# ShingoNishimoto/gnss_sim_receiver

Measured on AMD Instinct MI355X. Metric: IF Msamples/sec processed & tracked-channels sustained @1/2/4/8 GPU, higher is better.
Workload: dtype f32

## Files before the change

### gnss_sim_receiver_amd/csrc/trk_fast.hip

```cpp
#include <algorithm>
#include <cstdlib>
#include <type_traits>

#include "code_bits.h"
#include "corr_device.h"
#include "trk_engine.h"

#ifdef GNSSHIP_CORR_PROFILE
namespace gnsship {
namespace {
constexpr int kFProfEpochs = 16;
constexpr int kFProfFirst = 8;
constexpr int kFProfSlots = 88;
__device__ unsigned long long* g_trkf_prof = nullptr;
__shared__ int g_fprof_epoch;
__shared__ unsigned long long g_fprof_lds[kFProfEpochs * kFProfSlots];
#ifndef GNSSHIP_PROF_MASK
#define GNSSHIP_PROF_MASK 0xffffffffffffffffull
#endif
__device__ __forceinline__ constexpr bool prof_on(int k) { return ((GNSSHIP_PROF_MASK) >> (k < 63 ? k : 63)) & 1ull; }
__device__ __forceinline__ void trkf_prof_stamp(int e, int k)
{
    if (!prof_on(k)) return;
    const int r = e - kFProfFirst;
// ... 75 lines not shown
constexpr int acc_waves() { return (2 * NTT + 3) / 4; }
template <int NTT, int W>
constexpr int n_producers() { return W - 2 - acc_waves<NTT>(); }
constexpr int kMaxAccWaves = 4;
static_assert(kFWaves - 4 >= 1 && GNSSHIP_THRU_WAVES - 4 >= 1, "trk_fast needs at least one producer wave");
constexpr int kRoleControl = 0, kRoleReplay = 1, kRoleProducer = 2, kRoleAccum = 3;
#define GNSSHIP_PROBE(NAME)                                                  \
    do {                                                                     \
        _Pragma("unroll") for (int pr_ = 0; pr_ < (NAME); pr_++) __builtin_amdgcn_s_sleep(4); \
    } while (0)
#ifndef GNSSHIP_DELAY_ACC
#define GNSSHIP_DELAY_ACC 0
#endif
#ifndef GNSSHIP_DELAY_PROD
#define GNSSHIP_DELAY_PROD 0
#endif
#ifndef GNSSHIP_DELAY_REPLAY
#define GNSSHIP_DELAY_REPLAY 0
#endif
#ifndef GNSSHIP_DELAY_LOOP
#define GNSSHIP_DELAY_LOOP 0
#endif
#ifndef GNSSHIP_POLL_SLEEP
#define GNSSHIP_POLL_SLEEP 0
#endif
constexpr uint64_t kSlotEmpty = ~0ull;

struct FJob {
    int64_t off;
    float rem_code, code_step;
    float shifts[5];
    float dz_re, dz_im;
    float rem_carr, step;
    int32_t runnable, in_margin, M, S, tail, pad;
};

struct SpecArgs {
    double step_d, rate;
    int64_t if_num;
    float rem_prev;
    int32_t n_pred;
};

struct SpecPred {
    float rem, step, dz_re, dz_im;
};

struct FShared {
    FJob job;
    float taps[2][2 * kMaxTaps + 2];
    int32_t taps_seq[kMaxAccWaves];
    gnsship_trk_dump_record drec;
    double coh;
    int32_t seed_seq;
    int32_t job_seq;
    int32_t pre_seq;
    int32_t lock_seq;
    int32_t locked;
    int32_t tail_seq;
    int32_t acc_groups[kMaxAccWaves];
    int32_t step_seq;
    SpecArgs spec;
    SpecPred pred;
    int32_t pred_seq;
    int32_t verdict;
    f2 tailp[kAvxLanes][kMaxTaps + 1];
    double pre_pll[2], pre_dll[2];
    int32_t pll_seq, dll_seq;
};

__device__ __forceinline__ float unif(float v) { return __builtin_bit_cast(float, __builtin_amdgcn_readfirstlane(__builtin_bit_cast(int, v))); }
__device__ __forceinline__ FJob uniform_job(const FJob& s)
{
    FJob j;
    const uint64_t off = static_cast<uint64_t>(s.off);
    j.off = static_cast<int64_t>((static_cast<uint64_t>(static_cast<uint32_t>(__builtin_amdgcn_readfirstlane(static_cast<int>(off >> 32)))) << 32) |
                                 static_cast<uint32_t>(__builtin_amdgcn_readfirstlane(static_cast<int>(off & 0xffffffffu))));
    j.rem_code = unif(s.rem_code);
    j.code_step = unif(s.code_step);
    for (int t = 0; t < 5; t++) j.shifts[t] = unif(s.shifts[t]);
    j.dz_re = unif(s.dz_re);
    j.dz_im = unif(s.dz_im);
    j.rem_carr = unif(s.rem_carr);
    j.step = unif(s.step);
    j.runnable = __builtin_amdgcn_readfirstlane(s.runnable);
    j.in_margin = __builtin_amdgcn_readfirstlane(s.in_margin);
    j.M = __builtin_amdgcn_readfirstlane(s.M);
    j.S = __builtin_amdgcn_readfirstlane(s.S);
    j.tail = __builtin_amdgcn_readfirstlane(s.tail);
    j.pad = 0;
    return j;
}

__device__ __forceinline__ void store_slot(uint64_t* p, f2 z) { __hip_atomic_store(p, __builtin_bit_cast(uint64_t, z), __ATOMIC_RELAXED, __HIP_MEMORY_SCOPE_WORKGROUP); }
__device__ __forceinline__ uint64_t load_slot(const uint64_t* p) { return __hip_atomic_load(p, __ATOMIC_RELAXED, __HIP_MEMORY_SCOPE_WORKGROUP); }

__device__ __forceinline__ void publish_seq(int32_t* p, int v)
{
    __builtin_amdgcn_fence(__ATOMIC_RELEASE, "workgroup");
    __hip_atomic_store(p, v, __ATOMIC_RELAXED, __HIP_MEMORY_SCOPE_WORKGROUP);
}
__device__ __forceinline__ void wait_seq(int32_t* p, int need)
{
    while (__hip_atomic_load(p, __ATOMIC_RELAXED, __HIP_MEMORY_SCOPE_WORKGROUP) < need) __builtin_amdgcn_s_sleep(GNSSHIP_POLL_SLEEP);
    __builtin_amdgcn_fence(__ATOMIC_ACQUIRE, "workgroup");
}

__device__ __forceinline__ void lds_release_store(int32_t* p, int v)
{
    asm volatile("s_waitcnt lgkmcnt(0)" ::: "memory");
    __hip_atomic_store(p, v, __ATOMIC_RELAXED, __HIP_MEMORY_SCOPE_WORKGROUP);
}
__device__ __forceinline__ void lds_wait_eq(const int32_t* p, int v)
{
    while (__hip_atomic_load(p, __ATOMIC_RELAXED, __HIP_MEMORY_SCOPE_WORKGROUP) != v) __builtin_amdgcn_s_sleep(GNSSHIP_POLL_SLEEP);
    asm volatile("" ::: "memory");
}
__device__ __forceinline__ void lds_wait_ge(const int32_t* p, int v)
{
    while (__hip_atomic_load(p, __ATOMIC_RELAXED, __HIP_MEMORY_SCOPE_WORKGROUP) < v) __builtin_amdgcn_s_sleep(GNSSHIP_POLL_SLEEP);
    asm volatile("" ::: "memory");
}

// ... 688 lines not shown
    const int tail = N - kAvxLanes * M;
    const int n_groups = (S + 3) / 4;
    RChan rc;
    if (role == kRoleControl) rchan_load(sc, &sc, rc);
    KFast kf = make_kfast(k, sc.geo);
    __shared__ uint32_t sec_bits[kTrkMaxSecondary / 32], dsec_bits[kTrkMaxSecondary / 32];
    if constexpr (!THRU) {
        if (tid < kTrkMaxSecondary / 32) {
            sec_bits[tid] = kf.sv.secondary_bits[tid];
            dsec_bits[tid] = kf.sv.data_secondary_bits[tid];
        }
        kf.sv.secondary_bits = sec_bits;
        kf.sv.data_secondary_bits = dsec_bits;
        __syncthreads();
    }
    const auto& kp = loop_params<THRU>(k, kf);
    const bool pre_disc = __builtin_amdgcn_readfirstlane(GNSSHIP_PRE_DISC && !k.sync[sc.geo].secondary && k.sync[sc.geo].extend == 1 ? 1 : 0) != 0;
    uint64_t seed_start = 0;
    const uint64_t vl = k.conf.vector_length;
    const float spcf = static_cast<float>(k.code_samples_per_chip);
    const int32_t has_if = k.has_if;
    const double if_step = k.if_step_rad;
    float shv_w[5], shv_n[5];
    float smin_w = 0.0f, smax_w = 0.0f, smin_n = 0.0f, smax_n = 0.0f;
#pragma unroll
    for (int t = 0; t < 5; t++) {
        shv_w[t] = t < NT ? k.shifts[t] : 0.0f;
        shv_n[t] = t < NT ? k.shifts_n[t] : 0.0f;
        smin_w = fminf(smin_w, shv_w[t]);
        smax_w = fmaxf(smax_w, shv_w[t]);
        smin_n = fminf(smin_n, shv_n[t]);
        smax_n = fmaxf(smax_n, shv_n[t]);
    }
    auto code_fields = [&](FJob& j, uint64_t nir) __attribute__((always_inline)) {
        const bool nw = uni(rc.narrow) != 0;
        j.off = static_cast<int64_t>(nir - buf_first);
        j.rem_code = __fmul_rn(static_cast<float>(rc.rem_code_phase_chips), spcf);
        j.code_step = __fmul_rn(static_cast<float>(rc.code_phase_step_chips), spcf);
#pragma unroll
        for (int t = 0; t < 5; t++) j.shifts[t] = nw ? shv_n[t] : shv_w[t];
        const float smin = nw ? smin_n : smin_w, smax = nw ? smax_n : smax_w;
        const double span = static_cast<double>(j.code_step) * static_cast<double>(N > 0 ? N - 1 : 0);
        const double lo = fmin(0.0, span) + smin - j.rem_code - 2.0;
        const double hi = fmax(0.0, span) + smax - j.rem_code + 2.0;
        j.in_margin = (isfinite(lo) && isfinite(hi) && lo >= -kCodeMargin && hi < static_cast<double>(L + kCodeMargin)) ? 1 : 0;
        j.M = M;
        j.S = S;
        j.tail = tail;
    };
    auto make_seed = [&](int e) {
        const bool runnable = e < max_rounds && (rc.state == 2 || rc.state == 3 || rc.state == 4) && rc.nitems_read >= buf_first &&
                              rc.nitems_read + vl <= buf_first + static_cast<uint64_t>(buf_len);
        const float rem_carr = has_if ? static_cast<float>(fmod_2pi(static_cast<double>(rc.rem_carr_phase_rad) + kTwoPi * rc.if_cyc))
                                      : rc.rem_carr_phase_rad;
        const float stepf = static_cast<float>(rc.carrier_phase_step_rad + if_step);
        if (runnable) rc.epoch_start = rc.nitems_read;
        seed_start = rc.epoch_start;
        if (lane == 0) {
            FJob& j = sh.job;
            j.runnable = runnable ? 1 : 0;
            if (runnable) {
                code_fields(j, rc.nitems_read);
                j.rem_carr = rem_carr;
                j.step = stepf;
            }
            int code = 3;
            if (!SRING && __hip_atomic_load(&sh.pred_seq, __ATOMIC_RELAXED, __HIP_MEMORY_SCOPE_WORKGROUP) >= e + 1) {
                __builtin_amdgcn_fence(__ATOMIC_ACQUIRE, "workgroup");
                code = 2;
                if (runnable && __builtin_bit_cast(uint32_t, sh.pred.rem) == __builtin_bit_cast(uint32_t, rem_carr) &&
                    __builtin_bit_cast(uint32_t, sh.pred.step) == __builtin_bit_cast(uint32_t, stepf)) {
                    j.dz_re = sh.pred.dz_re;
                    j.dz_im = sh.pred.dz_im;
                    code = 1;
                }
            }
            sh.verdict = 4 * (e + 1) + code;
            publish_seq(&sh.seed_seq, e + 1);
            if (code == 1) publish_seq(&sh.job_seq, e + 1);
        }
    };
    if (role == kRoleControl) make_seed(0);
    int e_done = 0;
    bool cancel = false;
    if (role == kRoleReplay) {
        for (int e = 0;; e++) {
            FJob job;
                bool spec = false;
                SpecArgs sp{};
                while (__hip_atomic_load(&sh.seed_seq, __ATOMIC_RELAXED, __HIP_MEMORY_SCOPE_WORKGROUP) < e + 1) {
                    if (__hip_atomic_load(&sh.step_seq, __ATOMIC_RELAXED, __HIP_MEMORY_SCOPE_WORKGROUP) >= e + 1) {
                        sp.step_d = __builtin_bit_cast(double, uni64(__builtin_bit_cast(uint64_t, sh.spec.step_d)));
                        sp.rate = __builtin_bit_cast(double, uni64(__builtin_bit_cast(uint64_t, sh.spec.rate)));
                        sp.if_num = static_cast<int64_t>(uni64(static_cast<uint64_t>(sh.spec.if_num)));
                        sp.rem_prev = __builtin_bit_cast(float, __builtin_amdgcn_readfirstlane(__builtin_bit_cast(int, sh.spec.rem_prev)));
                        sp.n_pred = __builtin_amdgcn_readfirstlane(sh.spec.n_pred);
                        spec = true;
                        break;
                    }
                    __builtin_amdgcn_s_sleep(GNSSHIP_POLL_SLEEP);
                }
                __builtin_amdgcn_fence(__ATOMIC_ACQUIRE, "workgroup");
                GNSSHIP_FSTAMP(e, 0);
    #ifdef GNSSHIP_CORR_PROFILE
                if (lane == 0) g_fprof_epoch = e;
    #endif
                f2 zinit = f2{0.0f, 0.0f}, inc = f2{1.0f, 0.0f}, dz = f2{1.0f, 0.0f};
                float step_pre = 0.0f;
                bool published = false;
                float xl = 0.0f;
                if (spec) step_pre = static_cast<float>(sp.step_d + if_step);
                if (SRING && spec) derive_step(step_pre, inc, dz);
                if (!SRING && spec) {
                    float rem_pred = carr_rem_next(sp.rem_prev, carr_advance(sp.step_d, sp.rate, static_cast<double>(sp.n_pred)));
                    if (has_if) {
                        const int64_t ifn = (sp.if_num + kp.if_mod * static_cast<int64_t>(sp.n_pred)) % kp.fs_int;
                        const double ifc = static_cast<double>(ifn) / static_cast<double>(kp.fs_int);
                        rem_pred = static_cast<float>(fmod_2pi(static_cast<double>(rem_pred) + kTwoPi * ifc));
                    }
                    derive_all(step_pre, rem_pred, lane, inc, dz, zinit);
                    GNSSHIP_FSTAMP(e, 35);
                    GNSSHIP_PROBE(GNSSHIP_DELAY_REPLAY);
                    if (lane == 0) {
                        sh.pred.rem = rem_pred;
                        sh.pred.step = step_pre;
                        sh.pred.dz_re = dz.x;
                        sh.pred.dz_im = dz.y;
                        publish_seq(&sh.pred_seq, e + 1);
                    }
                    xl = (lane & 1) ? zinit.y : zinit.x;
                    if (lane < 2 * kAvxLanes) xl = fast_replay<G, false>(xl, dz.x, (lane & 1) ? dz.y : -dz.y, M, S, tail, Zs, rs, lane);
                    GNSSHIP_FSTAMP(e, 34);
                    wait_seq(&sh.seed_seq, e + 1);
                    const int v = __builtin_amdgcn_readfirstlane(sh.verdict);
                    int status = (v >> 2) == e + 1 ? (v & 3) : 3;
                    if (status == 3) {
                        const FJob sd = uniform_job(sh.job);
                        status = 2;
                        if (sd.runnable && __builtin_bit_cast(uint32_t, sd.step) == __builtin_bit_cast(uint32_t, step_pre) &&
                            __builtin_bit_cast(uint32_t, sd.rem_carr) == __builtin_bit_cast(uint32_t, rem_pred)) {
                            if (lane == 0) {
                                sh.job.dz_re = dz.x;
                                sh.job.dz_im = dz.y;
                                publish_seq(&sh.job_seq, e + 1);
                            }
                            status = 1;
                        }
                    }
                    GNSSHIP_FVAL(e, 78, static_cast<unsigned long long>(status));
                    if (status == 1) {
                        published = true;
                    } else {
                        for (int i = lane; i < S * kAvxLanes; i += kWave) Zs[i] = kSlotEmpty;
                    }
                    GNSSHIP_FSTAMP(e, 36);
                }
                if (!published) {
                    wait_seq(&sh.seed_seq, e + 1);
                    const FJob sd = uniform_job(sh.job);
                    if (sd.runnable) {
                        if (!(spec && __builtin_bit_cast(uint32_t, sd.step) == __builtin_bit_cast(uint32_t, step_pre))) derive_step(sd.step, inc, dz);
                        zinit = derive_chains(sd.rem_carr, inc, lane);
                        if (lane == 0) {
                            sh.job.dz_re = dz.x;
                            sh.job.dz_im = dz.y;
                        }
                    }
                    if (lane == 0) publish_seq(&sh.job_seq, e + 1);
                    if (!sd.runnable) break;
                }
                GNSSHIP_FSTAMP(e, 1);
                GNSSHIP_FCLK(e, 12);
                job = uniform_job(sh.job);
                if (!published) {
                    xl = (lane & 1) ? zinit.y : zinit.x;
                    if (lane < 2 * kAvxLanes) xl = fast_replay<G, SRING>(xl, job.dz_re, (lane & 1) ? job.dz_im : -job.dz_im, M, S, tail, Zs, rs, lane);
                }
                if (tail > 0) {
                    const i4v span = sample_span<FMT>(samples, job.off, N);
                    const f2 zl = f2{__builtin_bit_cast(float, __builtin_amdgcn_readlane(__builtin_bit_cast(int, xl), 0)),
                        __builtin_bit_cast(float, __builtin_amdgcn_readlane(__builtin_bit_cast(int, xl), 1))};
                    if (lane == 0) {
                        f2 p = normalise_avx(zl);
                        for (int j = 0; j < tail; j++) {
                            tailz[j] = p;
                            p = cmul_exact(p, inc);
                        }
                    }
                    if (job.in_margin)
                        fast_tail_products<FMT, NT, DATA, true, PACKED>(job, span, c0, c1, L, tailz, lane, sh.tailp);
                    else
                        fast_tail_products<FMT, NT, DATA, false, PACKED>(job, span, c0, c1, L, tailz, lane, sh.tailp);
                    if (lane == 0) publish_seq(&sh.tail_seq, e + 1);
                }
                GNSSHIP_FSTAMP(e, 2);
                GNSSHIP_FCLK(e, 13);
        }
    } else if (role == kRoleProducer) {
        f2 xa[G < 8 ? G : 8];
        float cv[G][NTT];
        for (int e = 0;; e++) {
            const int gbase = e * n_groups;
            wait_seq(&sh.job_seq, e + 1);
            const FJob job = uniform_job(sh.job);
            if (!job.runnable) break;
            const i4v span = sample_span<FMT>(samples, job.off, N);
            if (job.in_margin)
                fast_produce<FMT, NT, DATA, true, G, kFWaves, PACKED>(job, span, c0, c1, L, Zs, rs, Pp, rg, ready, sh.acc_groups, gbase, lane, pw, e, xa, cv);
            else
                fast_produce<FMT, NT, DATA, false, G, kFWaves, PACKED>(job, span, c0, c1, L, Zs, rs, Pp, rg, ready, sh.acc_groups, gbase, lane, pw, e, xa, cv);
            if (pw < 2) GNSSHIP_FSTAMP(e, 3 + pw);
            if (pw == 0) {
                wait_seq(&sh.pre_seq, e + 1);
                const double coh = sh.coh;
                if (lane == 0) {
                    GNSSHIP_TRK_LOOP_STAMP(8);
                    sh.locked = (coh > 0.0 && !lock_status(k, sc, coh)) ? 0 : 1;
                    GNSSHIP_TRK_LOOP_STAMP(26);
                    publish_seq(&sh.lock_seq, e + 1);
                }
            }
        }
    } else if (role == kRoleAccum) {
        for (int e = 0;; e++) {
            const int gbase = e * n_groups;
            wait_seq(&sh.job_seq, e + 1);
            const FJob job = uniform_job(sh.job);
            if (!job.runnable) break;
            {
                constexpr int NS = acc_slots<NTT>();
                float acc[NS];
                GNSSHIP_FSTAMP(e, 27);
                fast_accumulate<NTT, G>(Pp, rg, ready, &sh.acc_groups[pw], gbase, S, lane, pw, acc, e);
                GNSSHIP_FSTAMP(e, 5);
                const int r = lane >> 4;
    #pragma unroll
                for (int kk = 0; kk < NS; kk++) acc[kk] = avx_chain_sum(acc[kk]);
                if (job.tail > 0) {
                    wait_seq(&sh.tail_seq, e + 1);
                    for (int j = 0; j < job.tail; j++) {
    #pragma unroll
                        for (int kk = 0; kk < NS; kk++) {
                            const int sl = min(acc_slot<NTT>(pw, r, kk), 2 * NTT - 1);
                            const f2 tv = sh.tailp[j][sl >> 1];
                            acc[kk] = acc[kk] + ((sl & 1) ? tv.y : tv.x);
                        }
                    }
                }
                if ((lane & 15) == 0) {
    #pragma unroll
                    for (int kk = 0; kk < NS; kk++) {
                        const int sl = acc_slot<NTT>(pw, r, kk);
                        if (sl < 2 * NTT) {
                            const int tap = sl >> 1;
                            const int o = (DATA && tap == NT) ? 2 * kMaxTaps : 2 * tap;
                            sh.taps[e & 1][o + (sl & 1)] = acc[kk];
                        }
                    }
                }
                if (lane == 0) lds_release_store(&sh.taps_seq[pw], e + 1);
                if (pre_disc && pw < 2) {
#pragma unroll
                    for (int a = 0; a < NA; a++) wait_seq(&sh.taps_seq[a], e + 1);
                    const float* tp = sh.taps[e & 1];
                    const int eo = k.veml ? 2 : 0;
                    auto own = [&](int i) { return __fadd_rn(0.0f, __fmul_rn(1.0f, tp[i])); };
                    if (pw == 0 || NA == 1) {
                        const double v = pll_error_hz(k.track_pilot ? 0 : 1, own(eo + 2), own(eo + 3));
                        if (lane == 0) {
                            sh.pre_pll[e & 1] = v;
                            publish_seq(&sh.pll_seq, e + 1);
                        }
                    }
                    if (pw == 1 || NA == 1) {
                        const float ve[2] = {k.veml ? own(0) : 0.0f, k.veml ? own(1) : 0.0f};
                        const float ee[2] = {own(eo), own(eo + 1)};
                        const float ll[2] = {own(eo + 4), own(eo + 5)};
                        const float vl[2] = {k.veml ? own(8) : 0.0f, k.veml ? own(9) : 0.0f};
                        const double v = dll_error_chips(k, ve, ee, ll, vl, k.conf.early_late_space_chips);
                        if (lane == 0) {
                            sh.pre_dll[e & 1] = v;
                            publish_seq(&sh.dll_seq, e + 1);
                        }
                    }
                }
            }
            GNSSHIP_FSTAMP(e, 6);
        }
    } else {
        for (int e = 0;; e++) {
            const int gbase = e * n_groups;
            wait_seq(&sh.job_seq, e + 1);
            const FJob job = uniform_job(sh.job);
            if (!job.runnable) break;
#pragma unroll
            for (int a = 0; a < NA; a++) wait_seq(&sh.taps_seq[a], e + 1);
            GNSSHIP_FCLK(e, 14);
            if (cancel) {
                cancel = false;
                if (lane == 0) {
                    sh.coh = 0.0;
                    publish_seq(&sh.pre_seq, e + 1);
                }
                make_seed(e + 1);
                continue;
            }
            {
                const float* taps = sh.taps[e & 1];
                GNSSHIP_FSTAMP(e, 16);
                GNSSHIP_PROBE(GNSSHIP_DELAY_LOOP);
                const float* pdata = DATA ? taps + 2 * kMaxTaps : taps;
                gnsship_trk_epoch r{};
                r.flags = 8;
                gnsship_trk_dump_record* dr = dump ? &sh.drec : nullptr;
                const uint64_t es = rc.epoch_start;
                const double coh = epoch_pre(kp, rc, taps, pdata, r, nullptr, dr);
                GNSSHIP_FSTAMP(e, 17);
                if (lane == 0) {
                    sc.p[0] = rc.p[0];
                    sc.p[1] = rc.p[1];
                    sc.pull_in = rc.pull_in;
                    sh.coh = coh;
                    publish_seq(&sh.pre_seq, e + 1);
                }
                GNSSHIP_FSTAMP(e, 18);
                bool seeded = false;
                if (coh > 0.0) {
                    const double k_rcs = rc.rem_code_phase_samples, k_acc = rc.acc_carrier_phase_rad, k_dop = rc.carrier_doppler_hz;
                    const double k_cf = rc.code_freq_chips, k_rcc = rc.rem_code_phase_chips;
                    const float k_rem = rc.rem_carr_phase_rad;
                    const int32_t k_len = rc.current_prn_length_samples;
                    auto early_step = [&](double dop) {
                        if (rc.state == 4 && lane == 0) {
                            sh.spec.step_d = div_fs(kp, kTwoPi * dop);
                            sh.spec.rate = rc.carrier_phase_rate_step_rad;
                            sh.spec.if_num = rc.if_num;
                            sh.spec.rem_prev = rc.rem_carr_phase_rad;
                            sh.spec.n_pred = rc.current_prn_length_samples;
                            publish_seq(&sh.step_seq, e + 2);
                        }
                        GNSSHIP_FSTAMP(e, 32);
                    };
                    PreDisc pd{0.0, 0.0, 0};
                    if (pre_disc && r.state == 4 && __builtin_bit_cast(uint32_t, unif(rc.spc)) == __builtin_bit_cast(uint32_t, k.conf.early_late_space_chips)) {
                        wait_seq(&sh.pll_seq, e + 1);
                        wait_seq(&sh.dll_seq, e + 1);
                        pd.pll = sh.pre_pll[e & 1];
                        pd.dll = sh.pre_dll[e & 1];
                        pd.ok = 3;
                    }
                    epoch_loop(kp, rc, nullptr, early_step, &pd);
                    const uint64_t k_nir = rc.nitems_read;
                    const int64_t k_ifn = rc.if_num;
                    const double k_ifc = rc.if_cyc;
                    if (rc.state == 4) {
                        epoch_consume(kp, rc);
                        make_seed(e + 1);
                        GNSSHIP_FSTAMP(e, 33);
                        rc.epoch_start = es;
                        seeded = true;
                    }
                    wait_seq(&sh.lock_seq, e + 1);
                    GNSSHIP_FSTAMP(e, 19);
                    const bool locked = sh.locked != 0;
                    if (!locked) {
                        rc.rem_code_phase_samples = k_rcs;
                        rc.acc_carrier_phase_rad = k_acc;
                        rc.carrier_doppler_hz = k_dop;
                        rc.code_freq_chips = k_cf;
                        rc.rem_code_phase_chips = k_rcc;
                        rc.rem_carr_phase_rad = k_rem;
                        rc.current_prn_length_samples = k_len;
                        rc.nitems_read = k_nir;
                        rc.if_num = k_ifn;
                        rc.if_cyc = k_ifc;
                        cancel = seeded;
                    }
                    epoch_post(kp, rc, taps, pdata, r, locked, dr);
                }
                GNSSHIP_FSTAMP(e, 24);
                epoch_finish(kp, rc, r, !seeded);
                if (!seeded)
                    make_seed(e + 1);
                else if (!cancel)
                    rc.epoch_start = seed_start;
                GNSSHIP_FSTAMP(e, 25);
                if (lane == 0) {
                    const size_t slot = static_cast<size_t>(e) * n_chans + ch;
                    if (rec) rec[slot] = r;
                    if (dump && (r.flags & 16)) dump[slot] = sh.drec;
                    if (trace) {
                        gnsship_trk_corr_trace tr{};
                        tr.sample_counter = es;
                        tr.n_samples = N;
                        tr.n_taps = NT;
                        tr.rem_carrier_phase_rad = job.rem_carr;
                        tr.phase_step_rad = job.step;
                        tr.rem_code_phase_samples = job.rem_code;
                        tr.code_phase_step_samples = job.code_step;
                        for (int t = 0; t < 5; t++) tr.shifts[t] = job.shifts[t];
                        for (int t = 0; t < 10; t++) tr.taps[t] = t < 2 * NT ? taps[t] : 0.0f;
                        tr.data_prompt[0] = DATA ? pdata[0] : 0.0f;
                        tr.data_prompt[1] = DATA ? pdata[1] : 0.0f;
                        trace[slot] = tr;
                    }
                }
                e_done = e + 1;
                GNSSHIP_FSTAMP(e, 7);
                GNSSHIP_FCLK(e, 15);
            }
        }
// ... 173 lines not shown
```

### gnss_sim_receiver_amd/csrc/trk_loop.h

```cpp
#pragma once
#ifndef GNSSHIP_LOOP_INLINE
#define GNSSHIP_LOOP_INLINE
#endif
#include <cmath>
#include <type_traits>

#include "exact_div.h"
#include "trk_engine.h"

#ifndef GNSSHIP_TRK_LOOP_STAMP
#define GNSSHIP_TRK_LOOP_STAMP(k) ((void)0)
#endif

namespace gnsship {
namespace {


constexpr double kGnssPi = 3.1415926535898;
constexpr double kTwoPi = 2.0 * kGnssPi;
constexpr double kInvTwoPi = 1.0 / kTwoPi;
__device__ __forceinline__ double div_2pi(double x) { return div_by(x, kTwoPi, kInvTwoPi); }
__device__ __forceinline__ double fmod_2pi(double x) { return fmod_by(x, kTwoPi, kInvTwoPi); }
template <class K>
__device__ __forceinline__ double div_fs(const K& k, double x) { return div_by(x, k.conf.fs_in, k.inv_fs); }
// ... 663 lines not shown
    d->abs_L = hypotf_glibc(c.l[0], c.l[1]);
    d->abs_VL = k.veml ? hypotf_glibc(c.vl[0], c.vl[1]) : 0.0f;
    d->prompt_I = prompt[0];
    d->prompt_Q = prompt[1];
    d->PRN_start_sample_count = nir + static_cast<uint64_t>(c.current_prn_length_samples);
    d->acc_carrier_phase_rad = static_cast<float>(c.acc_carrier_phase_rad);
    d->carrier_doppler_hz = static_cast<float>(c.carrier_doppler_hz);
    d->carrier_doppler_rate_hz = static_cast<float>(c.carrier_phase_rate_step_rad * fs * fs / kTwoPi);
    d->code_freq_chips = static_cast<float>(c.code_freq_chips);
    d->code_freq_rate_chips = static_cast<float>(c.code_phase_rate_step_chips * fs * fs);
    d->carr_error_hz = static_cast<float>(c.carr_phase_error_hz);
    d->carr_error_filt_hz = static_cast<float>(c.carr_error_filt_hz);
    d->code_error_chips = static_cast<float>(c.code_error_chips);
    d->code_error_filt_chips = static_cast<float>(c.code_error_filt_chips);
    d->CN0_SNV_dB_Hz = mem(c).cn0_db_hz;
    d->carrier_lock_test = mem(c).carrier_lock_test;
    d->aux1 = static_cast<float>(c.rem_code_phase_samples);
    d->aux2 = static_cast<double>(nir + static_cast<uint64_t>(c.current_prn_length_samples));
    d->PRN = c.prn;
}

__device__ __forceinline__ bool seconds_exceed(uint64_t elapsed, uint32_t limit_s, uint64_t fs_int)
{
    return elapsed >= (static_cast<uint64_t>(limit_s) + 1u) * fs_int;
}

__device__ __forceinline__ int next_mod(int i, int n)
{
    const int v = i + 1;
    return v < n ? v : (v == n ? 0 : v % n);
}

template <class K, class C>
__device__ GNSSHIP_LOOP_INLINE double epoch_pre(const K& k, C& c, const float* taps, const float* pdata, gnsship_trk_epoch& rec, TrkHist* h,
    gnsship_trk_dump_record* dump)
{
    const uint64_t nir = c.epoch_start;
    const uint64_t fs_int = static_cast<uint64_t>(static_cast<int>(k.conf.fs_in));
    rec.sample_counter = nir;
    if (c.pull_in && seconds_exceed(nir - c.acq_sample_stamp, k.conf.pull_in_time_s, fs_int)) {
        c.pull_in = 0;
        mem(c).carrier_fail = 0;
        mem(c).code_fail = 0;
    }
    const int eo = k.veml ? 2 : 0;
    const int st = c.state;
    rec.state = st;
    if (st == 2) {
        if (k.veml) {
            c.ve[0] = taps[0];
            c.ve[1] = taps[1];
            c.vl[0] = taps[8];
            c.vl[1] = taps[9];
        }
        c.e[0] = taps[eo];
        c.e[1] = taps[eo + 1];
        c.p[0] = taps[eo + 2];
        c.p[1] = taps[eo + 3];
        c.l[0] = taps[eo + 4];
        c.l[1] = taps[eo + 5];
        c.spc = k.conf.early_late_space_chips;
        rec.prompt_i = static_cast<double>(c.p[0]);
        rec.prompt_q = static_cast<double>(c.p[1]);
        if (seconds_exceed(nir - c.acq_sample_stamp, k.conf.bit_synchronization_time_limit_s, fs_int)) mem(c).carrier_fail = 300000;
        return k.code_period;
    }
    float sgn = 1.0f;
    if (syncset(k, c).secondary) {
        sgn = bit_at(syncset(k, c).secondary_bits, c.current_symbol) ? -1.0f : 1.0f;
        c.current_symbol = next_mod(c.current_symbol, syncset(k, c).secondary_len);
    }
    if (k.veml) {
        cadd(c.ve, taps, sgn);
        cadd(c.vl, taps + 8, sgn);
    }
    cadd(c.e, taps + eo, sgn);
    cadd(c.p, taps + eo + 2, sgn);
    cadd(c.l, taps + eo + 4, sgn);
    const float* src = k.track_pilot ? pdata : taps + eo + 2;
    if (syncset(k, c).symbols_per_bit > 1) {
        if (syncset(k, c).data_secondary_len > 0) {
            cadd(c.p_data, src, bit_at(syncset(k, c).data_secondary_bits, c.current_data_symbol) ? -1.0f : 1.0f);
            c.current_data_symbol = next_mod(c.current_data_symbol, syncset(k, c).data_secondary_len);
        } else {
            cadd(c.p_data, src, 1.0f);
            c.current_data_symbol = next_mod(c.current_data_symbol, syncset(k, c).symbols_per_bit);
        }
    } else {
        c.p_data[0] = src[0];
        c.p_data[1] = src[1];
    }
    c.cloop = k.track_pilot ? 0 : 1;
    if (st == 3) {
        update_tracking_vars(k, c, h);
        if (c.current_data_symbol == 0) {
            log_data(k, c, taps, pdata, nir, dump);
            rec.flags |= 16;
            rec.prompt_i = static_cast<double>(c.p_data[0]);
            rec.prompt_q = static_cast<double>(c.p_data[1]);
            rec.flags |= 1;
            c.p_data[0] = c.p_data[1] = 0.0f;
        }
        c.ext_count++;
        if (c.ext_count == syncset(k, c).extend - 1) {
            c.ext_count = 0;
            c.state = 4;
        }
        return 0.0;
    }
    return k.code_period * static_cast<double>(syncset(k, c).extend);
}

template <class K, class C, class H = NoDopplerHook>
__device__ __forceinline__ void epoch_loop(const K& k, C& c, TrkHist* h, const H& on_doppler = H{}, const PreDisc* pre = nullptr)
{
    GNSSHIP_TRK_LOOP_STAMP(9);
    run_dll_pll(k, c, on_doppler, pre);
    GNSSHIP_TRK_LOOP_STAMP(10);
    update_tracking_vars(k, c, h);
    GNSSHIP_TRK_LOOP_STAMP(11);
}

template <class K, class C>
__device__ GNSSHIP_LOOP_INLINE void epoch_post(const K& k, C& c, const float* taps, const float* pdata, gnsship_trk_epoch& rec, bool locked,
    gnsship_trk_dump_record* dump)
// ... 119 lines not shown
```

Measured before the change: 667.6.

## Pack job record into vector LDS words and add steady-state fast path

The per-epoch job record in LDS is packed into two 16-byte vectors with flags bit-packed into the upper offset word. This cuts the number of LDS reads and readfirstlane operations each role wave performs. A steady-state path is added for locked state-4 tracking: the producer wave computes the lock test directly from the taps, and the loop wave skips epoch_pre and the pre_seq handshake. This shortens the critical inter-wave dependency chain per epoch, but it adds branching complexity and depends on the steady flag being computed correctly.

```diff
diff --git a/gnss_sim_receiver_amd/csrc/trk_fast.hip b/gnss_sim_receiver_amd/csrc/trk_fast.hip
--- a/gnss_sim_receiver_amd/csrc/trk_fast.hip
+++ b/gnss_sim_receiver_amd/csrc/trk_fast.hip
@@ -131,8 +131,28 @@
     float shifts[5];
     float dz_re, dz_im;
     float rem_carr, step;
-    int32_t runnable, in_margin, M, S, tail, pad;
+    int32_t runnable, in_margin, M, S, tail, steady;
+    int32_t narrow;
 };
+
+typedef uint32_t u4v __attribute__((ext_vector_type(4)));
+constexpr uint32_t kJobRunnable = 1u, kJobInMargin = 2u, kJobSteady = 4u, kJobNarrow = 8u;
+struct alignas(16) FJobLds {
+    uint32_t w[8];
+};
+__device__ __forceinline__ void job_store_a(FJobLds& s, int64_t off, uint32_t flags, float rem_code, float code_step)
+{
+    const uint64_t o = static_cast<uint64_t>(off);
+    *reinterpret_cast<u4v*>(&s.w[0]) = u4v{static_cast<uint32_t>(o), (static_cast<uint32_t>(o >> 32) & 0x00ffffffu) | (flags << 24),
+        __builtin_bit_cast(uint32_t, rem_code), __builtin_bit_cast(uint32_t, code_step)};
+}
+__device__ __forceinline__ void job_store_b(FJobLds& s, float rem_carr, float step, float dz_re, float dz_im)
+{
+    *reinterpret_cast<u4v*>(&s.w[4]) = u4v{__builtin_bit_cast(uint32_t, rem_carr), __builtin_bit_cast(uint32_t, step),
+        __builtin_bit_cast(uint32_t, dz_re), __builtin_bit_cast(uint32_t, dz_im)};
+}
+__device__ __forceinline__ void job_store_carr(FJobLds& s, float rem_carr, float step) { *reinterpret_cast<f2*>(&s.w[4]) = f2{rem_carr, step}; }
+__device__ __forceinline__ void job_store_dz(FJobLds& s, f2 dz) { *reinterpret_cast<f2*>(&s.w[6]) = dz; }
 
 struct SpecArgs {
     double step_d, rate;
@@ -141,12 +161,12 @@
     int32_t n_pred;
 };
 
-struct SpecPred {
+struct alignas(16) SpecPred {
     float rem, step, dz_re, dz_im;
 };
 
 struct FShared {
-    FJob job;
+    FJobLds job;
     float taps[2][2 * kMaxTaps + 2];
     int32_t taps_seq[kMaxAccWaves];
     gnsship_trk_dump_record drec;
@@ -169,25 +189,28 @@
 };
 
 __device__ __forceinline__ float unif(float v) { return __builtin_bit_cast(float, __builtin_amdgcn_readfirstlane(__builtin_bit_cast(int, v))); }
-__device__ __forceinline__ FJob uniform_job(const FJob& s)
+__device__ __forceinline__ FJob uniform_job(const FJobLds& s, int M, int S, int tail)
 {
     FJob j;
-    const uint64_t off = static_cast<uint64_t>(s.off);
-    j.off = static_cast<int64_t>((static_cast<uint64_t>(static_cast<uint32_t>(__builtin_amdgcn_readfirstlane(static_cast<int>(off >> 32)))) << 32) |
-                                 static_cast<uint32_t>(__builtin_amdgcn_readfirstlane(static_cast<int>(off & 0xffffffffu))));
-    j.rem_code = unif(s.rem_code);
-    j.code_step = unif(s.code_step);
-    for (int t = 0; t < 5; t++) j.shifts[t] = unif(s.shifts[t]);
-    j.dz_re = unif(s.dz_re);
-    j.dz_im = unif(s.dz_im);
-    j.rem_carr = unif(s.rem_carr);
-    j.step = unif(s.step);
-    j.runnable = __builtin_amdgcn_readfirstlane(s.runnable);
-    j.in_margin = __builtin_amdgcn_readfirstlane(s.in_margin);
-    j.M = __builtin_amdgcn_readfirstlane(s.M);
-    j.S = __builtin_amdgcn_readfirstlane(s.S);
-    j.tail = __builtin_amdgcn_readfirstlane(s.tail);
-    j.pad = 0;
+    const u4v a = *reinterpret_cast<const u4v*>(&s.w[0]), b = *reinterpret_cast<const u4v*>(&s.w[4]);
+    const uint32_t lo = __builtin_amdgcn_readfirstlane(a.x), hi = __builtin_amdgcn_readfirstlane(a.y);
+    j.off = static_cast<int64_t>((static_cast<uint64_t>(hi & 0x00ffffffu) << 32) | lo);
+    const uint32_t flags = hi >> 24;
+    j.rem_code = __builtin_bit_cast(float, __builtin_amdgcn_readfirstlane(a.z));
+    j.code_step = __builtin_bit_cast(float, __builtin_amdgcn_readfirstlane(a.w));
+    j.rem_carr = __builtin_bit_cast(float, __builtin_amdgcn_readfirstlane(b.x));
+    j.step = __builtin_bit_cast(float, __builtin_amdgcn_readfirstlane(b.y));
+    j.dz_re = __builtin_bit_cast(float, __builtin_amdgcn_readfirstlane(b.z));
+    j.dz_im = __builtin_bit_cast(float, __builtin_amdgcn_readfirstlane(b.w));
+    j.narrow = (flags & kJobNarrow) ? 1 : 0;
+#pragma unroll
+    for (int t = 0; t < 5; t++) j.shifts[t] = 0.0f;
+    j.runnable = (flags & kJobRunnable) ? 1 : 0;
+    j.in_margin = (flags & kJobInMargin) ? 1 : 0;
+    j.steady = (flags & kJobSteady) ? 1 : 0;
+    j.M = M;
+    j.S = S;
+    j.tail = tail;
     return j;
 }
 
@@ -942,22 +965,24 @@
         smin_n = fminf(smin_n, shv_n[t]);
         smax_n = fmaxf(smax_n, shv_n[t]);
     }
-    auto code_fields = [&](FJob& j, uint64_t nir) __attribute__((always_inline)) {
-        const bool nw = uni(rc.narrow) != 0;
-        j.off = static_cast<int64_t>(nir - buf_first);
-        j.rem_code = __fmul_rn(static_cast<float>(rc.rem_code_phase_chips), spcf);
-        j.code_step = __fmul_rn(static_cast<float>(rc.code_phase_step_chips), spcf);
-#pragma unroll
-        for (int t = 0; t < 5; t++) j.shifts[t] = nw ? shv_n[t] : shv_w[t];
-        const float smin = nw ? smin_n : smin_w, smax = nw ? smax_n : smax_w;
-        const double span = static_cast<double>(j.code_step) * static_cast<double>(N > 0 ? N - 1 : 0);
-        const double lo = fmin(0.0, span) + smin - j.rem_code - 2.0;
-        const double hi = fmax(0.0, span) + smax - j.rem_code + 2.0;
-        j.in_margin = (isfinite(lo) && isfinite(hi) && lo >= -kCodeMargin && hi < static_cast<double>(L + kCodeMargin)) ? 1 : 0;
-        j.M = M;
-        j.S = S;
-        j.tail = tail;
+    auto read_job = [&](float (&cur)[5], int& cur_nw) __attribute__((always_inline)) {
+        FJob j = uniform_job(sh.job, M, S, tail);
+        if constexpr (THRU) {
+#pragma unroll
+            for (int t = 0; t < 5; t++) j.shifts[t] = t < NT ? (j.narrow ? k.shifts_n[t] : k.shifts[t]) : 0.0f;
+            return j;
+        }
+        if (j.narrow != cur_nw) {
+#pragma unroll
+            for (int t = 0; t < 5; t++) cur[t] = t < NT ? (j.narrow ? k.shifts_n[t] : k.shifts[t]) : 0.0f;
+            cur_nw = j.narrow;
+        }
+#pragma unroll
+        for (int t = 0; t < 5; t++) j.shifts[t] = cur[t];
+        return j;
     };
+    constexpr bool kSteadyForm = !THRU && NT == 3 && !DATA;
+    const bool steady_run = kSteadyForm && pre_disc && !kp.conf.enable_fll_steady_state;
     auto make_seed = [&](int e) {
         const bool runnable = e < max_rounds && (rc.state == 2 || rc.state == 3 || rc.state == 4) && rc.nitems_read >= buf_first &&
                               rc.nitems_read + vl <= buf_first + static_cast<uint64_t>(buf_len);
@@ -966,25 +991,36 @@
         const float stepf = static_cast<float>(rc.carrier_phase_step_rad + if_step);
         if (runnable) rc.epoch_start = rc.nitems_read;
         seed_start = rc.epoch_start;
+        const bool steady = runnable && steady_run && rc.state == 4 && rc.pull_in == 0 &&
+                            __builtin_bit_cast(uint32_t, rc.spc) == __builtin_bit_cast(uint32_t, kp.conf.early_late_space_chips);
         if (lane == 0) {
-            FJob& j = sh.job;
-            j.runnable = runnable ? 1 : 0;
+            FJobLds& j = sh.job;
             if (runnable) {
-                code_fields(j, rc.nitems_read);
-                j.rem_carr = rem_carr;
-                j.step = stepf;
+                const bool nw = uni(rc.narrow) != 0;
+                const float rem_code = __fmul_rn(static_cast<float>(rc.rem_code_phase_chips), spcf);
+                const float code_step = __fmul_rn(static_cast<float>(rc.code_phase_step_chips), spcf);
+                const float smin = nw ? smin_n : smin_w, smax = nw ? smax_n : smax_w;
+                const double span = static_cast<double>(code_step) * static_cast<double>(N > 0 ? N - 1 : 0);
+                const double lo = fmin(0.0, span) + smin - rem_code - 2.0;
+                const double hi = fmax(0.0, span) + smax - rem_code + 2.0;
+                const bool in_margin = isfinite(lo) && isfinite(hi) && lo >= -kCodeMargin && hi < static_cast<double>(L + kCodeMargin);
+                const uint32_t flags = kJobRunnable | (in_margin ? kJobInMargin : 0u) | (steady ? kJobSteady : 0u) | (nw ? kJobNarrow : 0u);
+                job_store_a(j, static_cast<int64_t>(rc.nitems_read - buf_first), flags, rem_code, code_step);
+            } else {
+                job_store_a(j, 0, 0u, 0.0f, 0.0f);
             }
             int code = 3;
             if (!SRING && __hip_atomic_load(&sh.pred_seq, __ATOMIC_RELAXED, __HIP_MEMORY_SCOPE_WORKGROUP) >= e + 1) {
                 __builtin_amdgcn_fence(__ATOMIC_ACQUIRE, "workgroup");
                 code = 2;
-                if (runnable && __builtin_bit_cast(uint32_t, sh.pred.rem) == __builtin_bit_cast(uint32_t, rem_carr) &&
-                    __builtin_bit_cast(uint32_t, sh.pred.step) == __builtin_bit_cast(uint32_t, stepf)) {
-                    j.dz_re = sh.pred.dz_re;
-                    j.dz_im = sh.pred.dz_im;
+                const SpecPred pr = sh.pred;
+                if (runnable && __builtin_bit_cast(uint32_t, pr.rem) == __builtin_bit_cast(uint32_t, rem_carr) &&
+                    __builtin_bit_cast(uint32_t, pr.step) == __builtin_bit_cast(uint32_t, stepf)) {
+                    job_store_b(j, rem_carr, stepf, pr.dz_re, pr.dz_im);
                     code = 1;
                 }
             }
+            if (code != 1) job_store_carr(j, rem_carr, stepf);
             sh.verdict = 4 * (e + 1) + code;
             publish_seq(&sh.seed_seq, e + 1);
             if (code == 1) publish_seq(&sh.job_seq, e + 1);
@@ -994,6 +1030,8 @@
     int e_done = 0;
     bool cancel = false;
     if (role == kRoleReplay) {
+        float shc[5];
+        int sh_nw = -1;
         for (int e = 0;; e++) {
             FJob job;
                 bool spec = false;
@@ -1045,13 +1083,12 @@
                     const int v = __builtin_amdgcn_readfirstlane(sh.verdict);
                     int status = (v >> 2) == e + 1 ? (v & 3) : 3;
                     if (status == 3) {
-                        const FJob sd = uniform_job(sh.job);
+                        const FJob sd = read_job(shc, sh_nw);
                         status = 2;
                         if (sd.runnable && __builtin_bit_cast(uint32_t, sd.step) == __builtin_bit_cast(uint32_t, step_pre) &&
                             __builtin_bit_cast(uint32_t, sd.rem_carr) == __builtin_bit_cast(uint32_t, rem_pred)) {
                             if (lane == 0) {
-                                sh.job.dz_re = dz.x;
-                                sh.job.dz_im = dz.y;
+                                job_store_dz(sh.job, dz);
                                 publish_seq(&sh.job_seq, e + 1);
                             }
                             status = 1;
@@ -1067,21 +1104,18 @@
                 }
                 if (!published) {
                     wait_seq(&sh.seed_seq, e + 1);
-                    const FJob sd = uniform_job(sh.job);
+                    const FJob sd = read_job(shc, sh_nw);
                     if (sd.runnable) {
                         if (!(spec && __builtin_bit_cast(uint32_t, sd.step) == __builtin_bit_cast(uint32_t, step_pre))) derive_step(sd.step, inc, dz);
                         zinit = derive_chains(sd.rem_carr, inc, lane);
-                        if (lane == 0) {
-                            sh.job.dz_re = dz.x;
-                            sh.job.dz_im = dz.y;
-                        }
+                        if (lane == 0) job_store_dz(sh.job, dz);
                     }
                     if (lane == 0) publish_seq(&sh.job_seq, e + 1);
                     if (!sd.runnable) break;
                 }
                 GNSSHIP_FSTAMP(e, 1);
                 GNSSHIP_FCLK(e, 12);
-                job = uniform_job(sh.job);
+                job = read_job(shc, sh_nw);
                 if (!published) {
                     xl = (lane & 1) ? zinit.y : zinit.x;
                     if (lane < 2 * kAvxLanes) xl = fast_replay<G, SRING>(xl, job.dz_re, (lane & 1) ? job.dz_im : -job.dz_im, M, S, tail, Zs, rs, lane);
@@ -1109,10 +1143,14 @@
     } else if (role == kRoleProducer) {
         f2 xa[G < 8 ? G : 8];
         float cv[G][NTT];
+        bool lost = false;
+        float shc[5];
+        int sh_nw = -1;
+        const double coh_steady = k.code_period * static_cast<double>(k.sync[uni(sc.geo)].extend);
         for (int e = 0;; e++) {
             const int gbase = e * n_groups;
             wait_seq(&sh.job_seq, e + 1);
-            const FJob job = uniform_job(sh.job);
+            const FJob job = read_job(shc, sh_nw);
             if (!job.runnable) break;
             const i4v span = sample_span<FMT>(samples, job.off, N);
             if (job.in_margin)
@@ -1121,21 +1159,43 @@
                 fast_produce<FMT, NT, DATA, false, G, kFWaves, PACKED>(job, span, c0, c1, L, Zs, rs, Pp, rg, ready, sh.acc_groups, gbase, lane, pw, e, xa, cv);
             if (pw < 2) GNSSHIP_FSTAMP(e, 3 + pw);
             if (pw == 0) {
-                wait_seq(&sh.pre_seq, e + 1);
-                const double coh = sh.coh;
-                if (lane == 0) {
-                    GNSSHIP_TRK_LOOP_STAMP(8);
-                    sh.locked = (coh > 0.0 && !lock_status(k, sc, coh)) ? 0 : 1;
-                    GNSSHIP_TRK_LOOP_STAMP(26);
-                    publish_seq(&sh.lock_seq, e + 1);
+                bool locked = true;
+                if (kSteadyForm && job.steady) {
+#pragma unroll
+                    for (int a = 0; a < NA; a++) wait_seq(&sh.taps_seq[a], e + 1);
+                    if (lane == 0) {
+                        GNSSHIP_FSTAMP(e, 8);
+                        if (!lost) {
+                            const float* tp = sh.taps[e & 1] + (k.veml ? 2 : 0);
+                            sc.p[0] = __fadd_rn(0.0f, __fmul_rn(1.0f, tp[2]));
+                            sc.p[1] = __fadd_rn(0.0f, __fmul_rn(1.0f, tp[3]));
+                            locked = lock_status(k, sc, coh_steady);
+                        }
+                        sh.locked = locked ? 1 : 0;
+                        GNSSHIP_FSTAMP(e, 26);
+                        publish_seq(&sh.lock_seq, e + 1);
+                    }
+                } else {
+                    wait_seq(&sh.pre_seq, e + 1);
+                    const double coh = sh.coh;
+                    if (lane == 0) {
+                        GNSSHIP_FSTAMP(e, 8);
+                        locked = !(coh > 0.0 && !lock_status(k, sc, coh));
+                        sh.locked = locked ? 1 : 0;
+                        GNSSHIP_FSTAMP(e, 26);
+                        publish_seq(&sh.lock_seq, e + 1);
+                    }
                 }
+                lost = __builtin_amdgcn_readfirstlane(locked ? 0 : 1) != 0;
             }
         }
     } else if (role == kRoleAccum) {
+        float shc[5];
+        int sh_nw = -1;
         for (int e = 0;; e++) {
             const int gbase = e * n_groups;
             wait_seq(&sh.job_seq, e + 1);
-            const FJob job = uniform_job(sh.job);
+            const FJob job = read_job(shc, sh_nw);
             if (!job.runnable) break;
             {
                 constexpr int NS = acc_slots<NTT>();
@@ -1198,17 +1258,18 @@
             GNSSHIP_FSTAMP(e, 6);
         }
     } else {
+        float shc[5];
+        int sh_nw = -1;
         for (int e = 0;; e++) {
-            const int gbase = e * n_groups;
             wait_seq(&sh.job_seq, e + 1);
-            const FJob job = uniform_job(sh.job);
+            const FJob job = read_job(shc, sh_nw);
             if (!job.runnable) break;
 #pragma unroll
             for (int a = 0; a < NA; a++) wait_seq(&sh.taps_seq[a], e + 1);
             GNSSHIP_FCLK(e, 14);
             if (cancel) {
                 cancel = false;
-                if (lane == 0) {
+                if (!job.steady && lane == 0) {
                     sh.coh = 0.0;
                     publish_seq(&sh.pre_seq, e + 1);
                 }
@@ -1224,69 +1285,176 @@
                 r.flags = 8;
                 gnsship_trk_dump_record* dr = dump ? &sh.drec : nullptr;
                 const uint64_t es = rc.epoch_start;
-                const double coh = epoch_pre(kp, rc, taps, pdata, r, nullptr, dr);
-                GNSSHIP_FSTAMP(e, 17);
-                if (lane == 0) {
-                    sc.p[0] = rc.p[0];
-                    sc.p[1] = rc.p[1];
-                    sc.pull_in = rc.pull_in;
-                    sh.coh = coh;
-                    publish_seq(&sh.pre_seq, e + 1);
-                }
-                GNSSHIP_FSTAMP(e, 18);
                 bool seeded = false;
-                if (coh > 0.0) {
-                    const double k_rcs = rc.rem_code_phase_samples, k_acc = rc.acc_carrier_phase_rad, k_dop = rc.carrier_doppler_hz;
-                    const double k_cf = rc.code_freq_chips, k_rcc = rc.rem_code_phase_chips;
-                    const float k_rem = rc.rem_carr_phase_rad;
-                    const int32_t k_len = rc.current_prn_length_samples;
-                    auto early_step = [&](double dop) {
-                        if (rc.state == 4 && lane == 0) {
-                            sh.spec.step_d = div_fs(kp, kTwoPi * dop);
-                            sh.spec.rate = rc.carrier_phase_rate_step_rad;
-                            sh.spec.if_num = rc.if_num;
-                            sh.spec.rem_prev = rc.rem_carr_phase_rad;
-                            sh.spec.n_pred = rc.current_prn_length_samples;
-                            publish_seq(&sh.step_seq, e + 2);
-                        }
-                        GNSSHIP_FSTAMP(e, 32);
-                    };
-                    PreDisc pd{0.0, 0.0, 0};
-                    if (pre_disc && r.state == 4 && __builtin_bit_cast(uint32_t, unif(rc.spc)) == __builtin_bit_cast(uint32_t, k.conf.early_late_space_chips)) {
-                        wait_seq(&sh.pll_seq, e + 1);
-                        wait_seq(&sh.dll_seq, e + 1);
-                        pd.pll = sh.pre_pll[e & 1];
-                        pd.dll = sh.pre_dll[e & 1];
-                        pd.ok = 3;
-                    }
-                    epoch_loop(kp, rc, nullptr, early_step, &pd);
-                    const uint64_t k_nir = rc.nitems_read;
-                    const int64_t k_ifn = rc.if_num;
-                    const double k_ifc = rc.if_cyc;
-                    if (rc.state == 4) {
-                        epoch_consume(kp, rc);
-                        make_seed(e + 1);
-                        GNSSHIP_FSTAMP(e, 33);
-                        rc.epoch_start = es;
-                        seeded = true;
-                    }
-                    wait_seq(&sh.lock_seq, e + 1);
-                    GNSSHIP_FSTAMP(e, 19);
-                    const bool locked = sh.locked != 0;
-                    if (!locked) {
-                        rc.rem_code_phase_samples = k_rcs;
-                        rc.acc_carrier_phase_rad = k_acc;
-                        rc.carrier_doppler_hz = k_dop;
-                        rc.code_freq_chips = k_cf;
-                        rc.rem_code_phase_chips = k_rcc;
-                        rc.rem_carr_phase_rad = k_rem;
-                        rc.current_prn_length_samples = k_len;
-                        rc.nitems_read = k_nir;
-                        rc.if_num = k_ifn;
-                        rc.if_cyc = k_ifc;
-                        cancel = seeded;
-                    }
-                    epoch_post(kp, rc, taps, pdata, r, locked, dr);
+                if constexpr (kSteadyForm) {
+                    const bool steady = kSteadyForm && job.steady != 0;
+                    double coh = steady ? 1.0 : 0.0;
+                    double k_rcs = 0.0, k_acc = 0.0, k_dop = 0.0, k_cf = 0.0, k_rcc = 0.0, k_ifc = 0.0;
+                    float k_rem = 0.0f;
+                    int32_t k_len = 0;
+                    uint64_t k_nir = 0;
+                    int64_t k_ifn = 0;
+    #pragma unroll 1
+                    for (int pass = 0; pass < (kSteadyForm ? 2 : 1); pass++) {
+                        if ((pass == 1) == steady) {
+                            coh = epoch_pre(kp, rc, taps, pdata, r, nullptr, dr);
+                            GNSSHIP_FSTAMP(e, 17);
+                            if (!steady) {
+                                if (lane == 0) {
+                                    sc.p[0] = rc.p[0];
+                                    sc.p[1] = rc.p[1];
+                                    sc.pull_in = rc.pull_in;
+                                    sh.coh = coh;
+                                    publish_seq(&sh.pre_seq, e + 1);
+                                }
+                                GNSSHIP_FSTAMP(e, 18);
+                            }
+                        }
+                        if (pass == 0 && (steady || coh > 0.0)) {
+                            k_rcs = rc.rem_code_phase_samples;
+                            k_acc = rc.acc_carrier_phase_rad;
+                            k_dop = rc.carrier_doppler_hz;
+                            k_cf = rc.code_freq_chips;
+                            k_rcc = rc.rem_code_phase_chips;
+                            k_rem = rc.rem_carr_phase_rad;
+                            k_len = rc.current_prn_length_samples;
+                            PreDisc pd{0.0, 0.0, 0};
+                            if (steady || (pre_disc && r.state == 4 && __builtin_bit_cast(uint32_t, unif(rc.spc)) == __builtin_bit_cast(uint32_t, k.conf.early_late_space_chips))) {
+                                wait_seq(&sh.pll_seq, e + 1);
+                                pd.pll = sh.pre_pll[e & 1];
+                                pd.ok = 3;
+                                if constexpr (!kSteadyForm) {
+                                    wait_seq(&sh.dll_seq, e + 1);
+                                    pd.dll = sh.pre_dll[e & 1];
+                                }
+                            }
+                            auto early_step = [&](double dop) {
+                                if (rc.state == 4 && lane == 0) {
+                                    sh.spec.step_d = div_fs(kp, kTwoPi * dop);
+                                    sh.spec.rate = rc.carrier_phase_rate_step_rad;
+                                    sh.spec.if_num = rc.if_num;
+                                    sh.spec.rem_prev = rc.rem_carr_phase_rad;
+                                    sh.spec.n_pred = rc.current_prn_length_samples;
+                                    publish_seq(&sh.step_seq, e + 2);
+                                }
+                                GNSSHIP_FSTAMP(e, 32);
+                                if (kSteadyForm && pd.ok) {
+                                    wait_seq(&sh.dll_seq, e + 1);
+                                    pd.dll = sh.pre_dll[e & 1];
+                                }
+                            };
+                            epoch_loop(kp, rc, nullptr, early_step, &pd);
+                            k_nir = rc.nitems_read;
+                            k_ifn = rc.if_num;
+                            k_ifc = rc.if_cyc;
+                            if (rc.state == 4) {
+                                epoch_consume(kp, rc);
+                                make_seed(e + 1);
+                                GNSSHIP_FSTAMP(e, 33);
+                                rc.epoch_start = es;
+                                seeded = true;
+                            }
+                        }
+                    }
+                    if (coh > 0.0) {
+                        wait_seq(&sh.lock_seq, e + 1);
+                        GNSSHIP_FSTAMP(e, 19);
+                        const bool locked = sh.locked != 0;
+                        if (!locked) {
+                            rc.rem_code_phase_samples = k_rcs;
+                            rc.acc_carrier_phase_rad = k_acc;
+                            rc.carrier_doppler_hz = k_dop;
+                            rc.code_freq_chips = k_cf;
+                            rc.rem_code_phase_chips = k_rcc;
+                            rc.rem_carr_phase_rad = k_rem;
+                            rc.current_prn_length_samples = k_len;
+                            rc.nitems_read = k_nir;
+                            rc.if_num = k_ifn;
+                            rc.if_cyc = k_ifc;
+                            cancel = seeded;
+                        }
+                        epoch_post(kp, rc, taps, pdata, r, locked, dr);
+                    }
+                } else {
+                    const bool steady = kSteadyForm && job.steady != 0;
+                    double coh = 1.0;
+                    if (!steady) {
+                        coh = epoch_pre(kp, rc, taps, pdata, r, nullptr, dr);
+                        GNSSHIP_FSTAMP(e, 17);
+                        if (lane == 0) {
+                            sc.p[0] = rc.p[0];
+                            sc.p[1] = rc.p[1];
+                            sc.pull_in = rc.pull_in;
+                            sh.coh = coh;
+                            publish_seq(&sh.pre_seq, e + 1);
+                        }
+                        GNSSHIP_FSTAMP(e, 18);
+                    }
+                    if (coh > 0.0) {
+                        const double k_rcs = rc.rem_code_phase_samples, k_acc = rc.acc_carrier_phase_rad, k_dop = rc.carrier_doppler_hz;
+                        const double k_cf = rc.code_freq_chips, k_rcc = rc.rem_code_phase_chips;
+                        const float k_rem = rc.rem_carr_phase_rad;
+                        const int32_t k_len = rc.current_prn_length_samples;
+                        PreDisc pd{0.0, 0.0, 0};
+                        if (steady || (pre_disc && r.state == 4 && __builtin_bit_cast(uint32_t, unif(rc.spc)) == __builtin_bit_cast(uint32_t, k.conf.early_late_space_chips))) {
+                            wait_seq(&sh.pll_seq, e + 1);
+                            pd.pll = sh.pre_pll[e & 1];
+                            pd.ok = 3;
+                            if constexpr (THRU) {
+                                wait_seq(&sh.dll_seq, e + 1);
+                                pd.dll = sh.pre_dll[e & 1];
+                            }
+                        }
+                        auto early_step = [&](double dop) {
+                            if (rc.state == 4 && lane == 0) {
+                                sh.spec.step_d = div_fs(kp, kTwoPi * dop);
+                                sh.spec.rate = rc.carrier_phase_rate_step_rad;
+                                sh.spec.if_num = rc.if_num;
+                                sh.spec.rem_prev = rc.rem_carr_phase_rad;
+                                sh.spec.n_pred = rc.current_prn_length_samples;
+                                publish_seq(&sh.step_seq, e + 2);
+                            }
+                            GNSSHIP_FSTAMP(e, 32);
+                            if (!THRU && pd.ok) {
+                                wait_seq(&sh.dll_seq, e + 1);
+                                pd.dll = sh.pre_dll[e & 1];
+                            }
+                        };
+                        epoch_loop(kp, rc, nullptr, early_step, &pd);
+                        const uint64_t k_nir = rc.nitems_read;
+                        const int64_t k_ifn = rc.if_num;
+                        const double k_ifc = rc.if_cyc;
+                        if (rc.state == 4) {
+                            epoch_consume(kp, rc);
+                            make_seed(e + 1);
+                            GNSSHIP_FSTAMP(e, 33);
+                            rc.epoch_start = es;
+                            seeded = true;
+                        }
+                        if (steady) {
+                            r.sample_counter = es;
+                            r.state = 4;
+                            save_correlation_results(kp, rc, taps, pdata);
+                            GNSSHIP_FSTAMP(e, 81);
+                        }
+                        wait_seq(&sh.lock_seq, e + 1);
+                        GNSSHIP_FSTAMP(e, 19);
+                        const bool locked = sh.locked != 0;
+                        if (!locked) {
+                            rc.rem_code_phase_samples = k_rcs;
+                            rc.acc_carrier_phase_rad = k_acc;
+                            rc.carrier_doppler_hz = k_dop;
+                            rc.code_freq_chips = k_cf;
+                            rc.rem_code_phase_chips = k_rcc;
+                            rc.rem_carr_phase_rad = k_rem;
+                            rc.current_prn_length_samples = k_len;
+                            rc.nitems_read = k_nir;
+                            rc.if_num = k_ifn;
+                            rc.if_cyc = k_ifc;
+                            cancel = seeded;
+                        }
+                        epoch_post(kp, rc, taps, pdata, r, locked, dr);
+                    }
                 }
                 GNSSHIP_FSTAMP(e, 24);
                 epoch_finish(kp, rc, r, !seeded);
diff --git a/gnss_sim_receiver_amd/csrc/trk_loop.h b/gnss_sim_receiver_amd/csrc/trk_loop.h
--- a/gnss_sim_receiver_amd/csrc/trk_loop.h
+++ b/gnss_sim_receiver_amd/csrc/trk_loop.h
@@ -719,6 +719,38 @@
 }
 
 template <class K, class C>
+__device__ __forceinline__ void save_correlation_results(const K& k, C& c, const float* taps, const float* pdata)
+{
+    const int eo = k.veml ? 2 : 0;
+    float sgn = 1.0f;
+    if (syncset(k, c).secondary) {
+        sgn = bit_at(syncset(k, c).secondary_bits, c.current_symbol) ? -1.0f : 1.0f;
+        c.current_symbol = next_mod(c.current_symbol, syncset(k, c).secondary_len);
+    }
+    if (k.veml) {
+        cadd(c.ve, taps, sgn);
+        cadd(c.vl, taps + 8, sgn);
+    }
+    cadd(c.e, taps + eo, sgn);
+    cadd(c.p, taps + eo + 2, sgn);
+    cadd(c.l, taps + eo + 4, sgn);
+    const float* src = k.track_pilot ? pdata : taps + eo + 2;
+    if (syncset(k, c).symbols_per_bit > 1) {
+        if (syncset(k, c).data_secondary_len > 0) {
+            cadd(c.p_data, src, bit_at(syncset(k, c).data_secondary_bits, c.current_data_symbol) ? -1.0f : 1.0f);
+            c.current_data_symbol = next_mod(c.current_data_symbol, syncset(k, c).data_secondary_len);
+        } else {
+            cadd(c.p_data, src, 1.0f);
+            c.current_data_symbol = next_mod(c.current_data_symbol, syncset(k, c).symbols_per_bit);
+        }
+    } else {
+        c.p_data[0] = src[0];
+        c.p_data[1] = src[1];
+    }
+    c.cloop = k.track_pilot ? 0 : 1;
+}
+
+template <class K, class C>
 __device__ GNSSHIP_LOOP_INLINE double epoch_pre(const K& k, C& c, const float* taps, const float* pdata, gnsship_trk_epoch& rec, TrkHist* h,
     gnsship_trk_dump_record* dump)
 {
@@ -752,32 +784,7 @@
         if (seconds_exceed(nir - c.acq_sample_stamp, k.conf.bit_synchronization_time_limit_s, fs_int)) mem(c).carrier_fail = 300000;
         return k.code_period;
     }
-    float sgn = 1.0f;
-    if (syncset(k, c).secondary) {
-        sgn = bit_at(syncset(k, c).secondary_bits, c.current_symbol) ? -1.0f : 1.0f;
-        c.current_symbol = next_mod(c.current_symbol, syncset(k, c).secondary_len);
-    }
-    if (k.veml) {
-        cadd(c.ve, taps, sgn);
-        cadd(c.vl, taps + 8, sgn);
-    }
-    cadd(c.e, taps + eo, sgn);
-    cadd(c.p, taps + eo + 2, sgn);
-    cadd(c.l, taps + eo + 4, sgn);
-    const float* src = k.track_pilot ? pdata : taps + eo + 2;
-    if (syncset(k, c).symbols_per_bit > 1) {
-        if (syncset(k, c).data_secondary_len > 0) {
-            cadd(c.p_data, src, bit_at(syncset(k, c).data_secondary_bits, c.current_data_symbol) ? -1.0f : 1.0f);
-            c.current_data_symbol = next_mod(c.current_data_symbol, syncset(k, c).data_secondary_len);
-        } else {
-            cadd(c.p_data, src, 1.0f);
-            c.current_data_symbol = next_mod(c.current_data_symbol, syncset(k, c).symbols_per_bit);
-        }
-    } else {
-        c.p_data[0] = src[0];
-        c.p_data[1] = src[1];
-    }
-    c.cloop = k.track_pilot ? 0 : 1;
+    save_correlation_results(k, c, taps, pdata);
     if (st == 3) {
         update_tracking_vars(k, c, h);
         if (c.current_data_symbol == 0) {
```

Result: faster. 694.5, median of 6 (+4.0%).
